# nucypher/SGFHE.jl

Hardware: AMD Instinct MI355X
Metric: bootstraps/sec (higher is better)
Workload: dtype i32

## Files before the change

### sgfhe.jl_amd/csrc/kernels.h

```cpp
#pragma once

#include "ntt.h"

namespace sgfhe {

typedef unsigned __int128 u128;

constexpr int NPR_MAX = 7;
constexpr int LOGE = 4;

struct PrimeK {
    int32_t p;
    uint32_t pinv;
    int32_t sR;
    int32_t sRr;
    uint32_t hoff;
    int32_t r1, r2, r3;
    int32_t qmodp;
    int32_t kappaR;
    int32_t minvR;
    float invp;
    const int32_t *twf;
    const int32_t *twi;
    uint32_t npr;
// ... 131 lines not shown
    static_assert(ROUNDS % 2 == 0, "double rounds");
    const uint32_t s[16] = {0x61707865u, 0x3320646eu, 0x79622d32u, 0x6b206574u,
                            key.k[0], key.k[1], key.k[2], key.k[3],
                            key.k[4], key.k[5], key.k[6], key.k[7], c12, c13, c14, c15};
    uint32_t x[16];
#pragma unroll
    for (int i = 0; i < 16; i++) x[i] = s[i];
#define SGFHE_QR(a, b, c, d)                                                             \
    x[a] += x[b]; x[d] = __builtin_rotateleft32(x[d] ^ x[a], 16);                        \
    x[c] += x[d]; x[b] = __builtin_rotateleft32(x[b] ^ x[c], 12);                        \
    x[a] += x[b]; x[d] = __builtin_rotateleft32(x[d] ^ x[a], 8);                         \
    x[c] += x[d]; x[b] = __builtin_rotateleft32(x[b] ^ x[c], 7);
#pragma unroll
    for (int r = 0; r < ROUNDS / 2; r++) {
        SGFHE_QR(0, 4, 8, 12) SGFHE_QR(1, 5, 9, 13) SGFHE_QR(2, 6, 10, 14) SGFHE_QR(3, 7, 11, 15)
        SGFHE_QR(0, 5, 10, 15) SGFHE_QR(1, 6, 11, 12) SGFHE_QR(2, 7, 8, 13) SGFHE_QR(3, 4, 9, 14)
    }
#undef SGFHE_QR
#pragma unroll
    for (int i = 0; i < 16; i++) out[i] = x[i] + s[i];
}
struct RndRow {
    ChaChaKey key;
    uint32_t call, boot;
};
struct RndArgs {
    ChaChaKey key;
    uint32_t call, chunk;
    const RndRow *rows;
};
template <bool ROWS>
__device__ __forceinline__ void rnd_stream(const RndArgs &ra, uint32_t row, ChaChaKey &key, uint32_t &cz, uint32_t &cw) {
    if constexpr (ROWS) {
        const RndRow r = ra.rows[ra.chunk + row];
        key = r.key; cz = r.boot; cw = r.call;
    } else {
        key = ra.key; cz = ra.chunk + row; cw = ra.call;
    }
}
__device__ __forceinline__ uint4 rnd128(const ChaChaKey &key, uint4 ctr) {
    uint32_t w[16];
    chacha_block<RND_ROUNDS>(key, ctr.x >> 2, ctr.y, ctr.z, ctr.w, w);
    const uint32_t q = ctr.x & 3u;
    return make_uint4(q == 0 ? w[0] : q == 1 ? w[4] : q == 2 ? w[8] : w[12],
                      q == 0 ? w[1] : q == 1 ? w[5] : q == 2 ? w[9] : w[13],
                      q == 0 ? w[2] : q == 1 ? w[6] : q == 2 ? w[10] : w[14],
                      q == 0 ? w[3] : q == 1 ? w[7] : q == 2 ? w[11] : w[15]);
}
__device__ __forceinline__ ulonglong2 random_digits(u128 xn, const CrtConst *CC, const ChaChaKey &key,
                                                    uint4 ctr) {
    const uint4 rv = rnd128(key, ctr);
    const uint64_t span = 2 * CC->xmax + 1;
    const uint64_t r0 = (uint64_t)(((u128)(((uint64_t)rv.y << 32) | rv.x) * span) >> 64);
    const uint64_t r1 = (uint64_t)(((u128)(((uint64_t)rv.w << 32) | rv.z) * span) >> 64);
    const u128 B = CC->B, Q = CC->Q;
    const u128 tsub = mod_wide((u128)r1 * (uint64_t)B + r0, Q, CC->invQ, nullptr);
    const u128 x2 = xn >= tsub ? xn - tsub : xn + Q - tsub;
    uint64_t hi;
    const u128 lo = mod_wide(x2, B, CC->invB, &hi);
    return make_ulonglong2((uint64_t)lo + r0, hi + r1);
}

__device__ __forceinline__ int32_t digit_reduce(uint64_t e, const Mod &md, int32_t sR) {
    return sredc((int64_t)e, md) + sR;
}

__device__ __forceinline__ uint32_t handover_offset(const PrimeK &P) { return 3u * (uint32_t)P.p + P.hoff; }

template <int M, int E>
__device__ __forceinline__ void key_row_products(const int32_t (&x)[1][E], const int32_t *kp, int32_t *zp,
                                                 const Mod &md) {
#pragma unroll
    for (int h = 0; h < E / 4; h++) {
        const int4 a = reinterpret_cast<const int4 *>(kp)[h];
        const int4 bq = reinterpret_cast<const int4 *>(kp + M)[h];
        const int32_t ka[4] = {a.x, a.y, a.z, a.w};
        const int32_t kb[4] = {bq.x, bq.y, bq.z, bq.w};
        int32_t r0[4], r1[4];
#pragma unroll
        for (int t = 0; t < 4; t++) {
            const int32_t u = x[0][4 * h + t];
            r0[t] = smont(u, ka[t], md);
            r1[t] = smont(u, kb[t], md);
        }
        reinterpret_cast<int4 *>(zp)[h] = make_int4(r0[0], r0[1], r0[2], r0[3]);
        reinterpret_cast<int4 *>(zp + M)[h] = make_int4(r1[0], r1[1], r1[2], r1[3]);
    }
}
template <int M>
__device__ __forceinline__ void zpart_sum4(const int32_t *zp, int h, int32_t (&acc)[4]) {
    acc[0] = acc[1] = acc[2] = acc[3] = 0;
#pragma unroll
    for (int ph = 0; ph < 4; ph++) {
        const int4 v = reinterpret_cast<const int4 *>(zp + (size_t)ph * 2 * M)[h];
        acc[0] += v.x; acc[1] += v.y; acc[2] += v.z; acc[3] += v.w;
    }
}

struct QuarterHead {
    uint32_t q;
    int32_t wB, wP;
    __device__ __forceinline__ QuarterHead(uint32_t q_, const PrimeK &P)
        : q(q_), wB((q_ & 2) ? P.f3 : P.f2), wP((q_ & 2) ? P.fp3 : P.fp2) {}
    template <int MS>
    __device__ __forceinline__ int32_t point(const uint32_t *dl, const uint16_t *dh, uint32_t i, const PrimeK &P,
                                             const Mod &md, int32_t sRd) const {
        int32_t X[4];
#pragma unroll
        for (int t = 0; t < 4; t++)
            X[t] = digit_reduce(dl[i + t * MS] | ((uint64_t)dh[i + t * MS] << 32), md, sRd);
        const int32_t u = smont(X[2], P.f1, md);
        const int32_t a = (q & 2) ? X[0] - u : X[0] + u;
        const int32_t w = sredc((int64_t)X[1] * wB + (int64_t)X[3] * wP, md);
        return sred_floor((q & 1) ? a - w : a + w, md);
    }
};

template <int LOGM, int E>
__device__ __forceinline__ void rot_factors(int32_t (&dfac)[E], const PrimeK &P, uint32_t j, uint32_t q, int t) {
    constexpr uint32_t M = 1u << LOGM;
#pragma unroll
    for (int e = 0; e < E; e++) {
        const uint32_t sl = q * (M / 4) + (uint32_t)(E * t + e);
        const uint32_t br = __brev(sl) >> (32 - LOGM);
        dfac[e] = P.pw[(j * (2u * br + 1u)) & (2u * M - 1u)];
    }
}
__device__ __forceinline__ int32_t rot_centre(int32_t dfac, const PrimeK &P, const Mod &md) {
    return scentre(dfac - P.r1, md);
}

template <int NP>
__device__ __forceinline__ void quarter_residues(const int32_t *__restrict__ ypart, PrimeSet PS, uint32_t bc,
                                                 uint32_t i, uint32_t logm, uint32_t (&y)[NP]) {
    const uint32_t MS = (1u << logm) >> 2, jq = i & (MS - 1), qq = i >> (logm - 2);
#pragma unroll
    for (int q = 0; q < NP; q++) {
        const PrimeK P = PS[q];
        const Mod md = mod_of(P);
        const int32_t *yp = ypart + (((size_t)bc * NP + q) * 4) * MS + jq;
        int32_t r;
        if (qq & 1u) {
            const int32_t c1 = smont(yp[0] - yp[MS], P.v2, md), c3 = smont(yp[2 * MS] - yp[3 * MS], P.v3, md);
            r = (qq & 2u) ? smont(c1 - c3, P.v1, md) : c1 + c3;
        } else {
            const int32_t c0 = sred(yp[0] + yp[MS], md), c2 = sred(yp[2 * MS] + yp[3 * MS], md);
            r = (qq & 2u) ? smont(c0 - c2, P.v1, md) : c0 + c2;
        }
        y[q] = (uint32_t)r + handover_offset(P);
    }
}

constexpr int EXT_WAVES = 4;
constexpr int wide_split(int logm) { return logm >= 13 ? 2 : 4; }
constexpr int DET_SPLIT = 0;
constexpr int EXT_LE3_MAX = 9;
template <int LOGM, int LE, bool WIDE = false>
__global__ void __launch_bounds__((NttGeom<LOGM, LE>::T), (NttGeom<LOGM, LE>::T >= 256 ? EXT_WAVES : 1))
k_extprod(const uint64_t *__restrict__ dig, const int32_t *__restrict__ keyk,
          uint32_t *__restrict__ yres, const uint32_t *__restrict__ ua, PrimeSet PS, uint32_t k,
          uint32_t n, uint32_t mode) {
    using G = NttGeom<LOGM, LE>;
    constexpr int M = G::M, T = G::T, E = G::E;
    extern __shared__ __attribute__((aligned(16))) uint32_t lds[];
    int32_t *const z1 = reinterpret_cast<int32_t *>(lds) + M + threadIdx.x;

    const int tid = threadIdx.x;
    const uint32_t g = blockIdx.x;
    const uint32_t slot = g >> 3;
    const uint32_t npr = PS[0].npr;
    const uint32_t b = (slot / npr) * 8 + (g & 7);
    const uint32_t pi = slot % npr;
    const PrimeK P = PS[pi];
    const Mod md = mod_of(P);
    const uint32_t cpad = gridDim.x / npr;
    const BufRsrc rdig = make_rsrc(dig, cpad * 32u * (uint32_t)M);
    const BufRsrc rkey = make_rsrc(keyk, npr * 32u * (uint32_t)M);
#ifdef SGFHE_ABL_NO_YRES
    const BufRsrc ryres = make_rsrc(yres, 0u);
#else
    const BufRsrc ryres = make_rsrc(yres, cpad * npr * 8u * (uint32_t)M);
#endif

    const int32_t sRd = (mode & MODE_RANDOM) ? P.sRr : P.sR;
    constexpr int SPLIT = E == 16 ? (WIDE ? wide_split(LOGM) : DET_SPLIT) : 0;
    int64_t acc0[E];
#pragma unroll
    for (int e = 0; e < E; e++) { acc0[e] = 0; z1[e * T] = 0; }
#pragma unroll 1
    for (int ph = 0; ph < 4; ph++) {
        const int tid = (int)threadIdx.x + (int)opaque_zero();
        int32_t x[1][E];
        const uint32_t srec = (b * 2u + (uint32_t)(ph >> 1)) * 16u * (uint32_t)M;
        const uint32_t slo = srec + (uint32_t)(ph & 1) * 4u * (uint32_t)M;
        const uint32_t shi = srec + 8u * (uint32_t)M + (uint32_t)(ph & 1) * 2u * (uint32_t)M;
        const uint32_t vlo = 4u * (uint32_t)tid, vhi = 2u * (uint32_t)tid;
#pragma unroll
        for (int e = 0; e < E; e++) {
#ifdef SGFHE_ABL_NO_DIG
            x[0][e] = digit_reduce((uint64_t)(tid + e) * 0x9E3779B97F4Aull, md, sRd);
#else
            const uint32_t OL = (uint32_t)(4 * T * e), OH = (uint32_t)(2 * T * e);
            const uint32_t lo = buf_ld_u32(rdig, vlo + (OL & 4095u), slo + (OL & ~4095u));
            uint32_t hi = buf_ld_u16(rdig, vhi + (OH & 4095u), shi + (OH & ~4095u));
            if constexpr (WIDE)
                hi |= buf_ld_u8(rdig, (uint32_t)tid + ((uint32_t)(T * e) & 4095u),
                                srec + 12u * (uint32_t)M + (uint32_t)(ph & 1) * (uint32_t)M + ((uint32_t)(T * e) & ~4095u)) << 16;
            x[0][e] = digit_reduce(lo | ((uint64_t)hi << 32), md, sRd);
#endif
            if constexpr (SPLIT > 1)
                if ((e + 1) % (E / SPLIT) == 0 && e + 1 < E) __builtin_amdgcn_sched_barrier(0);
        }
        SGFHE_SYNC();

        const uint32_t skey = (pi * 8u + (uint32_t)ph * 2u) * 4u * (uint32_t)M;
        const uint32_t vkey = 4u * (uint32_t)E * (uint32_t)tid;
        int4 ka4[E / 4], kb4[E / 4];
        ntt_forward<LOGM, 1, LE>(x, lds, P.twf, tid, md);
#pragma unroll
        for (int h = 0; h < E / 4; h++) {
#ifdef SGFHE_ABL_NO_KEY
            ka4[h] = make_int4(tid, h, ph, 7), kb4[h] = make_int4(h, tid, 5, ph);
#else
            ka4[h] = buf_ld_i4(rkey, vkey + 16u * (uint32_t)h, skey);
            kb4[h] = buf_ld_i4(rkey, vkey + 16u * (uint32_t)h, skey + 4u * (uint32_t)M);
#endif
        }

        const Mod &mdp = md;
#pragma unroll
        for (int h = 0; h < E / 4; h++) {
            const int4 a = ka4[h], bq = kb4[h];
            const int32_t ka[4] = {a.x, a.y, a.z, a.w};
            const int32_t kb[4] = {bq.x, bq.y, bq.z, bq.w};
#pragma unroll
            for (int t = 0; t < 4; t++) {
                const int e = 4 * h + t;
                const int32_t u = x[0][e];
                acc0[e] += (int64_t)u * ka[t];
                int32_t *zp = reinterpret_cast<int32_t *>(lds) + M + e * T + tid;
                *zp += smont(u, kb[t], mdp);
            }
        }
    }
    int32_t z[2][E];
    constexpr bool WIDE0 = !inv_r4(LOGM) && LE == 4 && NttGeom<LOGM, LE>::SLAST_INV >= 0 &&
                           !(NttGeom<LOGM, LE>::RHO == 0 && NttGeom<LOGM, LE>::STOP == 0);
#pragma unroll
    for (int e = 0; e < E; e++) {
        const int32_t r0 = sredc(acc0[e], md);
        z[0][e] = WIDE0 ? r0 : sred(r0, md);
        z[1][e] = sred(z1[e * T], md);
    }
    SGFHE_SYNC();
    ntt_inverse<LOGM, 2, LE, WIDE0>(z, lds, P.twi, tid, md);

    const uint32_t sy0 = (b * 2u * npr + pi) * 4u * (uint32_t)M;
    const uint32_t sy1 = sy0 + npr * 4u * (uint32_t)M;
    const uint32_t vout = 4u * (uint32_t)tid;
    if (mode & MODE_PLAIN) {
#pragma unroll
        for (int c = 0; c < 2; c++)
#pragma unroll
            for (int e = 0; e < E; e++)
                buf_st_u32(ryres, vout + ((uint32_t)(4 * T * e) & 4095u),
                              (c ? sy1 : sy0) + ((uint32_t)(4 * T * e) & ~4095u),
                              condsub(sfull(z[c][e], md) + P.hoff, (uint32_t)P.p));
        return;
    }
    const uint32_t j = ua[(size_t)b * n + k];
    const uint32_t yoff = handover_offset(P);
    lds_store<LOGM, 2, LE, G::STOP>(z, lds, tid);
    SGFHE_SYNC();
    {
        constexpr uint32_t LOWMASK = (1u << G::STOP) - 1u;
        const uint32_t s0 = ((uint32_t)tid - j) & (2 * M - 1);
        const uint32_t lowswz = swz<LE>(s0 & LOWMASK);
        const uint32_t h0 = s0 >> G::STOP;
#pragma unroll
        for (int e = 0; e < E; e++) {
            const uint32_t he = h0 + e;
            const uint32_t hipart = (he & (E - 1)) << G::STOP;
            const uint32_t addr = hipart ^ lowswz ^ (G::STOP >= 9 ? 0u : swz_bits<LE>(hipart));
            const uint32_t smask = 0u - ((he >> LE) & 1u);
            const uint32_t yoe = yoff - smask;
#pragma unroll
            for (int c = 0; c < 2; c++) {
                const uint32_t v = lds[c * M + addr];
                const uint32_t y = (v ^ smask) + (yoe - (uint32_t)z[c][e]);
                buf_st_u32(ryres, vout + ((uint32_t)(4 * T * e) & 4095u),
                              (c ? sy1 : sy0) + ((uint32_t)(4 * T * e) & ~4095u), y);
            }
        }
    }
}

struct U96 {
    uint32_t w0, w1, w2;
};
__device__ __forceinline__ void mad96(U96 &a, uint32_t y, const uint32_t (&c)[3]) {
    const uint64_t p0 = (uint64_t)y * c[0] + a.w0;
    const uint64_t p1 = (uint64_t)y * c[1] + a.w1 + (p0 >> 32);
    a.w0 = (uint32_t)p0;
    a.w1 = (uint32_t)p1;
    a.w2 = y * c[2] + a.w2 + (uint32_t)(p1 >> 32);
}
template <int NP>
__device__ __forceinline__ U96 crt_reduce(const uint32_t (&y)[NP], const CrtConst *__restrict__ CC,
                                          bool have_old, ulonglong2 d) {
    float f = 0.f;
    double Sd = 0.0;
#pragma unroll
    for (int q = 0; q < NP; q++) {
        f += (float)y[q] * CC->invp[q];
#ifndef SGFHE_ABL_CRT_NOSD
        Sd += (double)y[q] * CC->cd[q];
#endif
    }
    const int alpha = (int)f;
    const uint4 tv = *reinterpret_cast<const uint4 *>(CC->T32[alpha]);
    U96 a = {tv.x, tv.y, tv.z};
    Sd += CC->Td[alpha];
#pragma unroll
    for (int q = 0; q < NP; q++) mad96(a, y[q], CC->c32[q]);
    if (have_old) {
        const uint64_t B = (uint64_t)CC->B;
        const uint32_t h0 = (uint32_t)d.y, h1 = (uint32_t)(d.y >> 32);
        const uint32_t b0 = (uint32_t)B, b1 = (uint32_t)(B >> 32);
        const uint64_t p0 = (uint64_t)h0 * b0 + a.w0 + (uint32_t)d.x;
        const uint64_t p1 = (uint64_t)h0 * b1 + (uint64_t)h1 * b0 + a.w1 + (uint32_t)(d.x >> 32) + (p0 >> 32);
        a.w0 = (uint32_t)p0;
        a.w1 = (uint32_t)p1;
        a.w2 += h1 * b1 + (uint32_t)(p1 >> 32);
#ifndef SGFHE_ABL_CRT_NOSD
        Sd += (double)d.y * CC->Bd + (double)d.x;
#endif
    }
    {
        const uint64_t q1 = (uint64_t)(Sd * CC->invQ);
        const uint32_t qa = (uint32_t)q1, qb = (uint32_t)(q1 >> 32);
        const uint64_t m0 = (uint64_t)qa * CC->Q32[0];
        const uint64_t m1 = (uint64_t)qa * CC->Q32[1] + (uint64_t)qb * CC->Q32[0] + (m0 >> 32);
        const uint32_t m2 = qa * CC->Q32[2] + qb * CC->Q32[1] + (uint32_t)(m1 >> 32);
        const uint64_t r0 = (uint64_t)a.w0 - (uint32_t)m0;
        const uint64_t r1 = (uint64_t)a.w1 - (uint32_t)m1 - ((r0 >> 32) & 1u);
        a.w2 = a.w2 - m2 - (uint32_t)((r1 >> 32) & 1u);
        a.w0 = (uint32_t)r0;
        a.w1 = (uint32_t)r1;
    }
    {
        const uint64_t Qlo = ((uint64_t)CC->Q32[1] << 32) | CC->Q32[0];
        const uint32_t Qhi = CC->Q32[2];
        uint64_t lo = ((uint64_t)a.w1 << 32) | a.w0;
        uint32_t hi = a.w2;
        if ((int32_t)hi < 0) {
            const uint64_t nlo = lo + Qlo;
            hi = hi + Qhi + (nlo < lo);
            lo = nlo;
        } else if (hi > Qhi || (hi == Qhi && lo >= Qlo)) {
            const uint64_t nlo = lo - Qlo;
            hi = hi - Qhi - (lo < Qlo);
            lo = nlo;
        }
        a.w0 = (uint32_t)lo;
        a.w1 = (uint32_t)(lo >> 32);
        a.w2 = hi;
    }
    return a;
}
template <int NP, bool ABLATE = false>
__device__ __forceinline__ void load_residues(const uint32_t *__restrict__ yres, uint32_t bc, uint32_t i,
                                              uint32_t logm, uint32_t (&y)[NP]) {
    const uint32_t yo = 4u * ((bc * NP << logm) + i);
#pragma unroll
    for (int q = 0; q < NP; q++) {
#ifdef SGFHE_ABL_NO_YRES
        if constexpr (ABLATE) { y[q] = (((bc << logm) + i) * 2654435761u + (uint32_t)q * 40503u) >> 3; continue; }
#endif
        y[q] = ld_off<uint32_t>(yres, yo + ((uint32_t)(4 * q) << logm));
    }
}
template <int NP, bool ABLATE = false>
__device__ __forceinline__ void load_residues4(const uint32_t *__restrict__ yres, uint32_t bc, uint32_t i,
                                               uint32_t logm, uint4 (&yv)[NP]) {
    typedef unsigned int v4u __attribute__((ext_vector_type(4)));
    const uint32_t yo = 4u * ((bc * NP << logm) + i);
#pragma unroll
    for (int q = 0; q < NP; q++) {
#ifdef SGFHE_ABL_NO_YLOAD
        if constexpr (ABLATE) { yv[q] = make_uint4((((bc << logm) + i) >> 2) + q, yo, i + 7u * q, bc); continue; }
#endif
        const v4u t = __builtin_nontemporal_load(reinterpret_cast<const v4u *>(
            reinterpret_cast<const char *>(yres) + yo + ((uint32_t)(4 * q) << logm)));
        yv[q] = make_uint4(t.x, t.y, t.z, t.w);
    }
}
template <int NP>
__device__ __forceinline__ void residues_of(const uint4 (&yv)[NP], int j, uint32_t (&y)[NP]) {
#pragma unroll
    for (int q = 0; q < NP; q++) y[q] = j == 0 ? yv[q].x : j == 1 ? yv[q].y : j == 2 ? yv[q].z : yv[q].w;
}

template <int NP, bool ROWS = false>
__global__ void __launch_bounds__(256)
k_crt_acc(const uint32_t *__restrict__ yres, uint64_t *__restrict__ dig,
          const CrtConst *__restrict__ CC, uint32_t total, uint32_t logm, uint32_t mode,
          RndArgs ra, uint32_t iter) {
    const uint32_t t = blockIdx.x * 256 + threadIdx.x;
// ... 1304 lines not shown
```

### sgfhe.jl_amd/csrc/ntt.h

```cpp
#pragma once

#include "rns_arith.h"

#ifdef SGFHE_ABL_NO_BARRIER
#define SGFHE_SYNC() ((void)0)
#else
#define SGFHE_SYNC() __syncthreads()
#endif

namespace sgfhe {

constexpr bool fwd_vec4(int logm) { return logm != 12 && logm != 14; }
constexpr bool inv_r4(int logm) { return logm != 12; }

template <int LOGE>
__host__ __device__ constexpr uint32_t swz_bits(uint32_t idx) {
    if constexpr (LOGE == 3)
        return (((idx >> 6) & 1u) * 0x09u) ^ (((idx >> 7) & 1u) * 0x12u) ^ (((idx >> 5) & 1u) * 0x04u);
    else
        return (((idx >> 5) & 1u) * 0x01u) ^ (((idx >> 6) & 1u) * 0x02u) ^
               (((idx >> 7) & 1u) * 0x04u) ^ (((idx >> 8) & 1u) * 0x18u);
}
template <int LOGE>
__host__ __device__ constexpr uint32_t swz(uint32_t idx) { return idx ^ swz_bits<LOGE>(idx); }

template <int LOGM, int LOGE>
struct NttGeom {
    static constexpr int M = 1 << LOGM;
    static constexpr int E = 1 << LOGE;
    static constexpr int T = M / E;
    static constexpr int RHO = LOGM % LOGE;
    static constexpr int STOP = LOGM - LOGE;
    static constexpr int SFIRST = RHO ? LOGM - RHO - LOGE : LOGM - 2 * LOGE;
    static constexpr int SLAST_INV = RHO ? LOGM - RHO - LOGE : STOP;
};

__device__ __forceinline__ uint32_t opaque_zero() {
    uint32_t z = 0;
    asm volatile("" : "+v"(z));
    return z;
}
__device__ __forceinline__ uint32_t opaque_zero_s() {
    uint32_t z = 0;
    asm volatile("" : "+s"(z));
    return z;
}

typedef __attribute__((address_space(4))) int32_t gmem_i32;


template <int LOGM, int LOGE, int S, int BHI, int BLO>
__device__ __forceinline__ void load_twiddles_at(int32_t (&t)[(1 << LOGE) - 1], const gmem_i32 *tw,
                                                 uint32_t hi) {
    constexpr int NG = 1 << (LOGE - 1 - BHI);
    const gmem_i32 *w = tw + (1u << (LOGM - 1 - S - BHI)) + (hi << (LOGE - 1 - BHI));
#pragma unroll
    for (int g = 0; g < NG; g++)
#ifdef SGFHE_ABL_NO_TW
        t[NG - 1 + g] = (int32_t)(hi + g + 12345u);
#else
        t[NG - 1 + g] = w[g];
#endif
    if constexpr (BHI > BLO) load_twiddles_at<LOGM, LOGE, S, BHI - 1, BLO>(t, tw, hi);
}
template <int LOGM, int LOGE, int S, int BHI, int BLO>
__device__ __forceinline__ void load_twiddles(int32_t (&t)[(1 << LOGE) - 1], const int32_t *tw,
                                              uint32_t hi) {
    if constexpr ((1 << S) >= 64) {
        const uint32_t hu = __builtin_amdgcn_readfirstlane(hi);
        load_twiddles_at<LOGM, LOGE, S, BHI, BLO>(t, (const gmem_i32 *)tw + opaque_zero_s(), hu);
    } else {
        load_twiddles_at<LOGM, LOGE, S, BHI, BLO>(t, (const gmem_i32 *)tw, hi);
    }
}


template <int NP, int LOGE, int B>
__device__ __forceinline__ void fwd_stage(int32_t (&x)[NP][1 << LOGE],
                                          const int32_t (&t)[(1 << LOGE) - 1], const Mod &md) {
    constexpr int NG = 1 << (LOGE - 1 - B);
#pragma unroll
    for (int q = 0; q < NP; q++)
#pragma unroll
        for (int g = 0; g < NG; g++)
#pragma unroll
            for (int l = 0; l < (1 << B); l++) {
                const int e0 = (g << (B + 1)) | l;
                bfly_fwd(x[q][e0], x[q][e0 | (1 << B)], t[NG - 1 + g], md);
            }
}
template <int NP, int LOGE, int BH>
__device__ __forceinline__ void fwd_step4(int32_t (&x)[NP][1 << LOGE], const int32_t (&t)[(1 << LOGE) - 1],
                                          const int32_t (&tp)[(1 << LOGE) - 1], const Mod &md) {
    static_assert(BH >= 1, "a radix-4 step covers local bits BH and BH - 1");
    constexpr int NGA = 1 << (LOGE - 1 - BH);
    constexpr int LO = 1 << (BH - 1), HI = 1 << BH;
#pragma unroll
    for (int q = 0; q < NP; q++)
#pragma unroll
        for (int g = 0; g < NGA; g++)
#pragma unroll
            for (int l = 0; l < LO; l++) {
                const int e0 = (g << (BH + 1)) | l;
                const int32_t wA = t[NGA - 1 + g];
                const int32_t wB0 = t[2 * NGA - 1 + 2 * g], wB1 = t[2 * NGA - 1 + 2 * g + 1];
                const int32_t P0 = tp[2 * NGA - 1 + 2 * g], P1 = tp[2 * NGA - 1 + 2 * g + 1];
                const int32_t X0 = x[q][e0], X1 = x[q][e0 | LO], X2 = x[q][e0 | HI], X3 = x[q][e0 | HI | LO];
                const int32_t u = smont(X2, wA, md);
                const int32_t a = X0 + u, b = X0 - u;
                const int32_t s_ = sredc((int64_t)X1 * wB0 + (int64_t)X3 * P0, md);
                const int32_t r_ = sredc((int64_t)X1 * wB1 + (int64_t)X3 * P1, md);
                x[q][e0] = a + s_;
                x[q][e0 | LO] = a - s_;
                x[q][e0 | HI] = b + r_;
                x[q][e0 | HI | LO] = b - r_;
            }
}
template <int NP, int LOGE, int BH>
__device__ __forceinline__ void fwd_reduce_x0(int32_t (&x)[NP][1 << LOGE], const Mod &md) {
#pragma unroll
    for (int q = 0; q < NP; q++)
#pragma unroll
        for (int e = 0; e < (1 << LOGE); e++)
            if ((e & (3 << (BH - 1))) == 0) x[q][e] = sred_floor(x[q][e], md);
}

template <int NP, int LOGE, int B>
__device__ __forceinline__ void inv_step4(int32_t (&x)[NP][1 << LOGE], const int32_t (&t)[(1 << LOGE) - 1],
                                          const int32_t (&tp)[(1 << LOGE) - 1], const Mod &md) {
    constexpr int NGA = 1 << (LOGE - 2 - B);
    constexpr int LO = 1 << B, HI = 1 << (B + 1);
#pragma unroll
    for (int q = 0; q < NP; q++)
#pragma unroll
        for (int g = 0; g < NGA; g++)
#pragma unroll
            for (int l = 0; l < LO; l++) {
                const int e0 = (g << (B + 2)) | l;
                const int32_t wA = t[NGA - 1 + g];
                const int32_t wB0 = t[2 * NGA - 1 + 2 * g], wB1 = t[2 * NGA - 1 + 2 * g + 1];
                const int32_t P0 = tp[2 * NGA - 1 + 2 * g], P1 = tp[2 * NGA - 1 + 2 * g + 1];
                const int32_t x0 = x[q][e0], x1 = x[q][e0 | LO], x2 = x[q][e0 | HI], x3 = x[q][e0 | HI | LO];
                const int32_t s0 = x0 + x1, s1 = x2 + x3, d0 = x0 - x1, d1 = x2 - x3;
                x[q][e0] = s0 + s1;
                x[q][e0 | HI] = smont(s0 - s1, wA, md);
                x[q][e0 | LO] = sredc((int64_t)d0 * wB0 + (int64_t)d1 * wB1, md);
                x[q][e0 | HI | LO] = sredc((int64_t)d0 * P0 + (int64_t)d1 * P1, md);
            }
}
template <int NP, int LOGE, int B>
__device__ __forceinline__ void inv_reduce_y0(int32_t (&x)[NP][1 << LOGE], const Mod &md) {
#pragma unroll
    for (int q = 0; q < NP; q++)
#pragma unroll
        for (int e = 0; e < (1 << LOGE); e++)
            if ((e & (3 << B)) == 0) x[q][e] = sred(x[q][e], md);
}

template <int NP, int LOGE, int B, uint32_t REDMASK, uint32_t REDMASK0>
__device__ __forceinline__ void inv_stage(int32_t (&x)[NP][1 << LOGE],
                                          const int32_t (&t)[(1 << LOGE) - 1], const Mod &md) {
    constexpr int NG = 1 << (LOGE - 1 - B);
#pragma unroll
    for (int q = 0; q < NP; q++)
#pragma unroll
        for (int g = 0; g < NG; g++)
#pragma unroll
            for (int l = 0; l < (1 << B); l++) {
                const int e0 = (g << (B + 1)) | l;
                bfly_inv(x[q][e0], x[q][e0 | (1 << B)], t[NG - 1 + g], md,
                         (((q == 0 ? REDMASK0 : REDMASK) >> e0) & 1u) != 0);
            }
}

template <int NP, int LOGE, int BHI, int BLO>
__device__ __forceinline__ void fwd_stages(int32_t (&x)[NP][1 << LOGE],
                                           const int32_t (&t)[(1 << LOGE) - 1], const Mod &md) {
    fwd_stage<NP, LOGE, BHI>(x, t, md);
    if constexpr (BHI > BLO) fwd_stages<NP, LOGE, BHI - 1, BLO>(x, t, md);
}
template <int NP, int LOGE>
__device__ __forceinline__ void fwd_reduce_x(int32_t (&x)[NP][1 << LOGE], const Mod &md) {
#pragma unroll
    for (int q = 0; q < NP; q++)
#pragma unroll
        for (int e = 0; e < (1 << (LOGE - 1)); e++) x[q][e] = sred_floor(x[q][e], md);
}
template <int LOGE, int B, int BLO, int BHI, int BFIRST, int LASTRED>
constexpr uint32_t inv_red_mask() {
    if (LOGE == 4 && BFIRST == 0 && BHI == 3 && LASTRED) {
        uint32_t m = 0;
        for (int e0 = 0; e0 < 16; e0++) {
            if (e0 & (1 << B)) continue;
            bool red = false;
            if (LASTRED == 3)
                red = B == 0 || B == 3 || (B == 2 && (e0 & 2) == 0);
            else
                red = B == 1 ? (e0 & 1) == 0
                    : B == 2 ? (e0 & 3) == 1
                    : B == 3 ? (LASTRED == 2 ? (e0 == 0 || e0 == 2 || e0 == 3) : true) : false;
            if (red) m |= 1u << e0;
        }
        return m;
    }
    return ((((B - BFIRST) & 1) != 0) || (LASTRED && B == BHI)) ? 0xFFFFFFFFu : 0u;
}
template <int NP, int LOGE, int BLO, int BHI, int BFIRST, int LASTRED, int LASTRED0 = LASTRED>
__device__ __forceinline__ void inv_stages(int32_t (&x)[NP][1 << LOGE],
                                           const int32_t (&t)[(1 << LOGE) - 1], const Mod &md) {
    inv_stage<NP, LOGE, BLO, inv_red_mask<LOGE, BLO, BLO, BHI, BFIRST, LASTRED>(),
              inv_red_mask<LOGE, BLO, BLO, BHI, BFIRST, LASTRED0>()>(x, t, md);
    if constexpr (BLO < BHI) inv_stages<NP, LOGE, BLO + 1, BHI, BFIRST, LASTRED, LASTRED0>(x, t, md);
}


template <int LOGE, int S>
__device__ __forceinline__ uint32_t lds_base(int tid) {
    const uint32_t lo = (uint32_t)tid & ((1u << S) - 1u);
    const uint32_t hi = (uint32_t)tid >> S;
    return swz<LOGE>((hi << (S + LOGE)) | lo);
}
template <int LOGM, int NP, int LOGE, int S>
__device__ __forceinline__ void lds_store(const int32_t (&x)[NP][1 << LOGE], uint32_t *lds, int tid) {
#ifdef SGFHE_ABL_NO_LDS
    return;
#endif
    constexpr int M = 1 << LOGM;
    const uint32_t pb = lds_base<LOGE, S>(tid) << 2;
    char *const base = reinterpret_cast<char *>(lds);
#pragma unroll
    for (int e = 0; e < (1 << LOGE); e++) {
        const uint32_t a = pb ^ (swz<LOGE>((uint32_t)e << S) << 2);
#pragma unroll
        for (int q = 0; q < NP; q++) *reinterpret_cast<int32_t *>(base + q * M * 4 + a) = x[q][e];
    }
}
template <int LOGM, int NP, int LOGE, int S>
__device__ __forceinline__ void lds_load(int32_t (&x)[NP][1 << LOGE], const uint32_t *lds, int tid) {
#ifdef SGFHE_ABL_NO_LDS
    return;
#endif
    constexpr int M = 1 << LOGM;
    const uint32_t pb = lds_base<LOGE, S>(tid) << 2;
    const char *const base = reinterpret_cast<const char *>(lds);
#pragma unroll
    for (int e = 0; e < (1 << LOGE); e++) {
        const uint32_t a = pb ^ (swz<LOGE>((uint32_t)e << S) << 2);
#pragma unroll
        for (int q = 0; q < NP; q++) x[q][e] = *reinterpret_cast<const int32_t *>(base + q * M * 4 + a);
    }
}


template <int LOGE, int SLOW>
__device__ __forceinline__ void exchange_sync() {
#ifdef SGFHE_ABL_ONEBAR
    if constexpr ((SLOW == 0 || SLOW == LOGE) && (1 << LOGE) <= 64) {
#else
    if constexpr (SLOW == 0 && (1 << LOGE) <= 64) {
#endif
#ifndef SGFHE_ABL_NO_BARRIER
        __builtin_amdgcn_fence(__ATOMIC_RELEASE, "wavefront");
#endif
    } else {
        SGFHE_SYNC();
    }
}

template <int LOGM, int NP, int LOGE, int SPREV, int SCUR>
struct FwdPasses {
    static __device__ __forceinline__ void run(int32_t (&x)[NP][1 << LOGE], uint32_t *lds,
                                               const int32_t *tw, int tid, const Mod &md) {
        int32_t t[(1 << LOGE) - 1], tp[(1 << LOGE) - 1];
        load_twiddles<LOGM, LOGE, SCUR, LOGE - 1, 0>(t, tw, (uint32_t)tid >> SCUR);
        constexpr bool UNIFORM = (1 << SCUR) >= 64;
        constexpr bool TWO_STEPS = LOGE == 4 && UNIFORM;
        if constexpr (UNIFORM || fwd_vec4(LOGM)) {
            load_twiddles<LOGM, LOGE, SCUR, LOGE - 2, LOGE - 2>(tp, tw + (2 << LOGM), (uint32_t)tid >> SCUR);
            if constexpr (TWO_STEPS) load_twiddles<LOGM, LOGE, SCUR, 0, 0>(tp, tw + (2 << LOGM), (uint32_t)tid >> SCUR);
        }
        lds_store<LOGM, NP, LOGE, SPREV>(x, lds, tid);
        exchange_sync<LOGE, SCUR>();
        lds_load<LOGM, NP, LOGE, SCUR>(x, lds, tid);
        Mod mdl = md;
        mdl.negp += (int32_t)opaque_zero_s();
        if constexpr (TWO_STEPS) {
            fwd_reduce_x0<NP, LOGE, 3>(x, mdl);
            fwd_step4<NP, LOGE, 3>(x, t, tp, mdl);
            fwd_reduce_x0<NP, LOGE, 1>(x, mdl);
            fwd_step4<NP, LOGE, 1>(x, t, tp, mdl);
        } else if constexpr (UNIFORM || fwd_vec4(LOGM)) {
            fwd_reduce_x<NP, LOGE>(x, mdl);
            fwd_step4<NP, LOGE, LOGE - 1>(x, t, tp, mdl);
            fwd_stages<NP, LOGE, LOGE - 3, 0>(x, t, mdl);
        } else {
            fwd_reduce_x<NP, LOGE>(x, mdl);
            fwd_stages<NP, LOGE, LOGE - 1, 0>(x, t, mdl);
        }
        if constexpr (SCUR >= LOGE)
            FwdPasses<LOGM, NP, LOGE, SCUR, SCUR - LOGE>::run(x, lds, tw, tid, md);
    }
};
template <int LOGM, int LOGE, int S>
__device__ __forceinline__ void load_inv_products(int32_t (&tp)[(1 << LOGE) - 1], const int32_t *tw, int tid) {
    if constexpr (inv_r4(LOGM)) {
        load_twiddles<LOGM, LOGE, S, 0, 0>(tp, tw + (2 << LOGM), (uint32_t)tid >> S);
        if constexpr (LOGE == 4 && (1 << S) >= 64)
            load_twiddles<LOGM, LOGE, S, 2, 2>(tp, tw + (2 << LOGM), (uint32_t)tid >> S);
    }
}
template <int LOGM, int NP, int LOGE, int SCUR, int SLAST, bool FINAL = false, bool WIDE0 = false>
struct InvPasses {
    static __device__ __forceinline__ void run(int32_t (&x)[NP][1 << LOGE], uint32_t *lds,
                                               const int32_t *tw, int tid, const Mod &md,
                                               const int32_t (&t)[(1 << LOGE) - 1],
                                               const int32_t (&tp)[(1 << LOGE) - 1]) {
        constexpr int MODE = (FINAL && SCUR == SLAST) ? 2 : 1;
        if constexpr (!inv_r4(LOGM)) {
            static_assert(!WIDE0 || (LOGE == 4 && !(FINAL && SLAST == 0)), "wide first pass: radix 16, not the final pass");
            inv_stages<NP, LOGE, 0, LOGE - 1, 0, MODE, (WIDE0 && SCUR == 0) ? 3 : MODE>(x, t, md);
        } else {
            static_assert(!WIDE0, "the radix-4 inverse takes every polynomial below 0.75 * 2^29");
            constexpr bool UNIFORM = (1 << SCUR) >= 64;
            inv_step4<NP, LOGE, 0>(x, t, tp, md);
            inv_reduce_y0<NP, LOGE, 0>(x, md);
            if constexpr (LOGE == 4 && UNIFORM) {
                inv_step4<NP, LOGE, 2>(x, t, tp, md);
                inv_reduce_y0<NP, LOGE, 2>(x, md);
            } else if constexpr (LOGE == 4) {
                inv_stage<NP, LOGE, 2, 0u, 0u>(x, t, md);
                inv_stage<NP, LOGE, 3, MODE == 2 ? 0x000Fu : 0x00FFu, MODE == 2 ? 0x000Fu : 0x00FFu>(x, t, md);
            } else {
                static_assert(LOGE == 3, "8 or 16 points per thread");
                inv_stage<NP, LOGE, 2, MODE == 2 ? 0u : 0x0Fu, MODE == 2 ? 0u : 0x0Fu>(x, t, md);
            }
        }
        if constexpr (SCUR < SLAST) {
            int32_t tn[(1 << LOGE) - 1], tpn[(1 << LOGE) - 1];
            load_twiddles<LOGM, LOGE, SCUR + LOGE, LOGE - 1, 0>(tn, tw,
                                                                (uint32_t)tid >> (SCUR + LOGE));
            load_inv_products<LOGM, LOGE, SCUR + LOGE>(tpn, tw, tid);
            lds_store<LOGM, NP, LOGE, SCUR>(x, lds, tid);
            exchange_sync<LOGE, SCUR>();
            lds_load<LOGM, NP, LOGE, SCUR + LOGE>(x, lds, tid);
            InvPasses<LOGM, NP, LOGE, SCUR + LOGE, SLAST, FINAL, WIDE0>::run(x, lds, tw, tid, md, tn, tpn);
        }
    }
};

template <int LOGM, int NP, int LOGE>
__device__ __forceinline__ void ntt_forward(int32_t (&x)[NP][1 << LOGE], uint32_t *lds,
                                            const int32_t *tw, int tid, const Mod &md) {
    using G = NttGeom<LOGM, LOGE>;
    constexpr int BLO = G::RHO == 0 ? 0 : LOGE - G::RHO;
    int32_t t[(1 << LOGE) - 1];
    load_twiddles<LOGM, LOGE, G::STOP, LOGE - 1, BLO>(t, tw, 0u);
    fwd_stages<NP, LOGE, LOGE - 1, BLO>(x, t, md);
    if constexpr (G::SFIRST >= 0)
        FwdPasses<LOGM, NP, LOGE, G::STOP, G::SFIRST>::run(x, lds, tw, tid, md);
}

template <int LOGM, int NP, int LOGE, bool WIDE0 = false>
__device__ __forceinline__ void ntt_inverse(int32_t (&x)[NP][1 << LOGE], uint32_t *lds,
                                            const int32_t *tw, int tid, const Mod &md) {
    using G = NttGeom<LOGM, LOGE>;
    if constexpr (G::RHO == 0) {
        int32_t t[(1 << LOGE) - 1], tp[(1 << LOGE) - 1];
        load_twiddles<LOGM, LOGE, 0, LOGE - 1, 0>(t, tw, (uint32_t)tid);
        load_inv_products<LOGM, LOGE, 0>(tp, tw, tid);
        InvPasses<LOGM, NP, LOGE, 0, G::STOP, true, WIDE0>::run(x, lds, tw, tid, md, t, tp);
    } else {
        int32_t tp[(1 << LOGE) - 1];
        if constexpr (G::SLAST_INV >= 0) {
            int32_t t[(1 << LOGE) - 1], tq[(1 << LOGE) - 1];
            load_twiddles<LOGM, LOGE, 0, LOGE - 1, 0>(t, tw, (uint32_t)tid);
            load_inv_products<LOGM, LOGE, 0>(tq, tw, tid);
            InvPasses<LOGM, NP, LOGE, 0, G::SLAST_INV, false, WIDE0>::run(x, lds, tw, tid, md, t, tq);
            load_twiddles<LOGM, LOGE, G::STOP, LOGE - 1, LOGE - G::RHO>(tp, tw, 0u);
            lds_store<LOGM, NP, LOGE, G::SLAST_INV>(x, lds, tid);
            SGFHE_SYNC();
            lds_load<LOGM, NP, LOGE, G::STOP>(x, lds, tid);
        } else {
            load_twiddles<LOGM, LOGE, G::STOP, LOGE - 1, LOGE - G::RHO>(tp, tw, 0u);
        }
        inv_stages<NP, LOGE, LOGE - G::RHO, LOGE - 1, LOGE - G::RHO, 0>(x, tp, md);
    }
}

}
```

Baseline: 2141.

## Process digit pairs per forward NTT, keep both accumulators in registers

The external-product kernel now loads two digit polynomials per iteration and runs a two-polynomial forward NTT, halving the outer loop from four phases to two. Both output accumulators stay in 32-bit registers, each updated by one Montgomery reduction per pair of products, instead of one 64-bit register accumulator plus one accumulator held in LDS. Key loads are double-buffered in groups with scheduling barriers. The WIDE0 lazy-reduction path in the inverse NTT is removed. This trades LDS traffic and barriers for more register pressure, which may reduce occupancy.

```diff
diff --git a/sgfhe.jl_amd/csrc/kernels.h b/sgfhe.jl_amd/csrc/kernels.h
--- a/sgfhe.jl_amd/csrc/kernels.h
+++ b/sgfhe.jl_amd/csrc/kernels.h
@@ -307,8 +307,7 @@
 }
 
 constexpr int EXT_WAVES = 4;
-constexpr int wide_split(int logm) { return logm >= 13 ? 2 : 4; }
-constexpr int DET_SPLIT = 0;
+constexpr int pair_split(int e, bool wide) { return e == 16 && wide ? 2 : 0; }
 constexpr int EXT_LE3_MAX = 9;
 template <int LOGM, int LE, bool WIDE = false>
 __global__ void __launch_bounds__((NttGeom<LOGM, LE>::T), (NttGeom<LOGM, LE>::T >= 256 ? EXT_WAVES : 1))
@@ -318,7 +317,6 @@
     using G = NttGeom<LOGM, LE>;
     constexpr int M = G::M, T = G::T, E = G::E;
     extern __shared__ __attribute__((aligned(16))) uint32_t lds[];
-    int32_t *const z1 = reinterpret_cast<int32_t *>(lds) + M + threadIdx.x;
 
     const int tid = threadIdx.x;
     const uint32_t g = blockIdx.x;
@@ -338,77 +336,81 @@
 #endif
 
     const int32_t sRd = (mode & MODE_RANDOM) ? P.sRr : P.sR;
-    constexpr int SPLIT = E == 16 ? (WIDE ? wide_split(LOGM) : DET_SPLIT) : 0;
-    int64_t acc0[E];
-#pragma unroll
-    for (int e = 0; e < E; e++) { acc0[e] = 0; z1[e * T] = 0; }
+    constexpr int SPLIT = pair_split(E, WIDE);
+    int32_t acc[2][E];
+#pragma unroll
+    for (int e = 0; e < E; e++) acc[0][e] = acc[1][e] = 0;
 #pragma unroll 1
-    for (int ph = 0; ph < 4; ph++) {
+    for (int pp = 0; pp < 2; pp++) {
         const int tid = (int)threadIdx.x + (int)opaque_zero();
-        int32_t x[1][E];
-        const uint32_t srec = (b * 2u + (uint32_t)(ph >> 1)) * 16u * (uint32_t)M;
-        const uint32_t slo = srec + (uint32_t)(ph & 1) * 4u * (uint32_t)M;
-        const uint32_t shi = srec + 8u * (uint32_t)M + (uint32_t)(ph & 1) * 2u * (uint32_t)M;
+        int32_t x[2][E];
+        const uint32_t srec = (b * 2u + (uint32_t)pp) * 16u * (uint32_t)M;
         const uint32_t vlo = 4u * (uint32_t)tid, vhi = 2u * (uint32_t)tid;
 #pragma unroll
         for (int e = 0; e < E; e++) {
+#pragma unroll
+            for (int r = 0; r < 2; r++) {
 #ifdef SGFHE_ABL_NO_DIG
-            x[0][e] = digit_reduce((uint64_t)(tid + e) * 0x9E3779B97F4Aull, md, sRd);
+                x[r][e] = digit_reduce((uint64_t)(tid + e + 16 * r) * 0x9E3779B97F4Aull, md, sRd);
 #else
-            const uint32_t OL = (uint32_t)(4 * T * e), OH = (uint32_t)(2 * T * e);
-            const uint32_t lo = buf_ld_u32(rdig, vlo + (OL & 4095u), slo + (OL & ~4095u));
-            uint32_t hi = buf_ld_u16(rdig, vhi + (OH & 4095u), shi + (OH & ~4095u));
-            if constexpr (WIDE)
-                hi |= buf_ld_u8(rdig, (uint32_t)tid + ((uint32_t)(T * e) & 4095u),
-                                srec + 12u * (uint32_t)M + (uint32_t)(ph & 1) * (uint32_t)M + ((uint32_t)(T * e) & ~4095u)) << 16;
-            x[0][e] = digit_reduce(lo | ((uint64_t)hi << 32), md, sRd);
+                const uint32_t slo = srec + (uint32_t)r * 4u * (uint32_t)M;
+                const uint32_t shi = srec + 8u * (uint32_t)M + (uint32_t)r * 2u * (uint32_t)M;
+                const uint32_t OL = (uint32_t)(4 * T * e), OH = (uint32_t)(2 * T * e);
+                const uint32_t lo = buf_ld_u32(rdig, vlo + (OL & 4095u), slo + (OL & ~4095u));
+                uint32_t hi = buf_ld_u16(rdig, vhi + (OH & 4095u), shi + (OH & ~4095u));
+                if constexpr (WIDE)
+                    hi |= buf_ld_u8(rdig, (uint32_t)tid + ((uint32_t)(T * e) & 4095u),
+                                    srec + 12u * (uint32_t)M + (uint32_t)r * (uint32_t)M + ((uint32_t)(T * e) & ~4095u)) << 16;
+                x[r][e] = digit_reduce(lo | ((uint64_t)hi << 32), md, sRd);
 #endif
+            }
             if constexpr (SPLIT > 1)
                 if ((e + 1) % (E / SPLIT) == 0 && e + 1 < E) __builtin_amdgcn_sched_barrier(0);
         }
         SGFHE_SYNC();
 
-        const uint32_t skey = (pi * 8u + (uint32_t)ph * 2u) * 4u * (uint32_t)M;
+        ntt_forward<LOGM, 2, LE>(x, lds, P.twf, tid, md);
+        const uint32_t skey = (pi * 8u + (uint32_t)pp * 4u) * 4u * (uint32_t)M;
         const uint32_t vkey = 4u * (uint32_t)E * (uint32_t)tid;
-        int4 ka4[E / 4], kb4[E / 4];
-        ntt_forward<LOGM, 1, LE>(x, lds, P.twf, tid, md);
+
+        __builtin_amdgcn_sched_barrier(0);
+        int4 kq[2][2][2];
+        const auto key_group = [&](int4 (&kg)[2][2], int h) {
+#pragma unroll
+            for (int r = 0; r < 2; r++)
+#pragma unroll
+                for (int c = 0; c < 2; c++)
+#ifdef SGFHE_ABL_NO_KEY
+                    kg[r][c] = make_int4(tid + r, h + c, pp, 7);
+#else
+                    kg[r][c] = buf_ld_i4(rkey, vkey + 16u * (uint32_t)h, skey + (uint32_t)(2 * r + c) * 4u * (uint32_t)M);
+#endif
+        };
+        key_group(kq[0], 0);
 #pragma unroll
         for (int h = 0; h < E / 4; h++) {
-#ifdef SGFHE_ABL_NO_KEY
-            ka4[h] = make_int4(tid, h, ph, 7), kb4[h] = make_int4(h, tid, 5, ph);
-#else
-            ka4[h] = buf_ld_i4(rkey, vkey + 16u * (uint32_t)h, skey);
-            kb4[h] = buf_ld_i4(rkey, vkey + 16u * (uint32_t)h, skey + 4u * (uint32_t)M);
-#endif
+            if (h + 1 < E / 4) key_group(kq[(h + 1) & 1], h + 1);
+            const int4 (&kg)[2][2] = kq[h & 1];
+#pragma unroll
+            for (int c = 0; c < 2; c++) {
+                const int32_t k0[4] = {kg[0][c].x, kg[0][c].y, kg[0][c].z, kg[0][c].w};
+                const int32_t k1[4] = {kg[1][c].x, kg[1][c].y, kg[1][c].z, kg[1][c].w};
+#pragma unroll
+                for (int t = 0; t < 4; t++) {
+                    const int e = 4 * h + t;
+                    acc[c][e] += sredc((int64_t)x[0][e] * k0[t] + (int64_t)x[1][e] * k1[t], md);
+                }
+            }
+            __builtin_amdgcn_sched_barrier(0);
         }
-
-        const Mod &mdp = md;
-#pragma unroll
-        for (int h = 0; h < E / 4; h++) {
-            const int4 a = ka4[h], bq = kb4[h];
-            const int32_t ka[4] = {a.x, a.y, a.z, a.w};
-            const int32_t kb[4] = {bq.x, bq.y, bq.z, bq.w};
-#pragma unroll
-            for (int t = 0; t < 4; t++) {
-                const int e = 4 * h + t;
-                const int32_t u = x[0][e];
-                acc0[e] += (int64_t)u * ka[t];
-                int32_t *zp = reinterpret_cast<int32_t *>(lds) + M + e * T + tid;
-                *zp += smont(u, kb[t], mdp);
-            }
-        }
     }
     int32_t z[2][E];
-    constexpr bool WIDE0 = !inv_r4(LOGM) && LE == 4 && NttGeom<LOGM, LE>::SLAST_INV >= 0 &&
-                           !(NttGeom<LOGM, LE>::RHO == 0 && NttGeom<LOGM, LE>::STOP == 0);
 #pragma unroll
     for (int e = 0; e < E; e++) {
-        const int32_t r0 = sredc(acc0[e], md);
-        z[0][e] = WIDE0 ? r0 : sred(r0, md);
-        z[1][e] = sred(z1[e * T], md);
-    }
-    SGFHE_SYNC();
-    ntt_inverse<LOGM, 2, LE, WIDE0>(z, lds, P.twi, tid, md);
+        z[0][e] = sred(acc[0][e], md);
+        z[1][e] = sred(acc[1][e], md);
+    }
+    ntt_inverse<LOGM, 2, LE>(z, lds, P.twi, tid, md);
 
     const uint32_t sy0 = (b * 2u * npr + pi) * 4u * (uint32_t)M;
     const uint32_t sy1 = sy0 + npr * 4u * (uint32_t)M;
diff --git a/sgfhe.jl_amd/csrc/ntt.h b/sgfhe.jl_amd/csrc/ntt.h
--- a/sgfhe.jl_amd/csrc/ntt.h
+++ b/sgfhe.jl_amd/csrc/ntt.h
@@ -157,7 +157,7 @@
             if ((e & (3 << B)) == 0) x[q][e] = sred(x[q][e], md);
 }
 
-template <int NP, int LOGE, int B, uint32_t REDMASK, uint32_t REDMASK0>
+template <int NP, int LOGE, int B, uint32_t REDMASK>
 __device__ __forceinline__ void inv_stage(int32_t (&x)[NP][1 << LOGE],
                                           const int32_t (&t)[(1 << LOGE) - 1], const Mod &md) {
     constexpr int NG = 1 << (LOGE - 1 - B);
@@ -169,7 +169,7 @@
             for (int l = 0; l < (1 << B); l++) {
                 const int e0 = (g << (B + 1)) | l;
                 bfly_inv(x[q][e0], x[q][e0 | (1 << B)], t[NG - 1 + g], md,
-                         (((q == 0 ? REDMASK0 : REDMASK) >> e0) & 1u) != 0);
+                         ((REDMASK >> e0) & 1u) != 0);
             }
 }
 
@@ -192,25 +192,20 @@
         uint32_t m = 0;
         for (int e0 = 0; e0 < 16; e0++) {
             if (e0 & (1 << B)) continue;
-            bool red = false;
-            if (LASTRED == 3)
-                red = B == 0 || B == 3 || (B == 2 && (e0 & 2) == 0);
-            else
-                red = B == 1 ? (e0 & 1) == 0
-                    : B == 2 ? (e0 & 3) == 1
-                    : B == 3 ? (LASTRED == 2 ? (e0 == 0 || e0 == 2 || e0 == 3) : true) : false;
+            const bool red = B == 1 ? (e0 & 1) == 0
+                           : B == 2 ? (e0 & 3) == 1
+                           : B == 3 ? (LASTRED == 2 ? (e0 == 0 || e0 == 2 || e0 == 3) : true) : false;
             if (red) m |= 1u << e0;
         }
         return m;
     }
     return ((((B - BFIRST) & 1) != 0) || (LASTRED && B == BHI)) ? 0xFFFFFFFFu : 0u;
 }
-template <int NP, int LOGE, int BLO, int BHI, int BFIRST, int LASTRED, int LASTRED0 = LASTRED>
+template <int NP, int LOGE, int BLO, int BHI, int BFIRST, int LASTRED>
 __device__ __forceinline__ void inv_stages(int32_t (&x)[NP][1 << LOGE],
                                            const int32_t (&t)[(1 << LOGE) - 1], const Mod &md) {
-    inv_stage<NP, LOGE, BLO, inv_red_mask<LOGE, BLO, BLO, BHI, BFIRST, LASTRED>(),
-              inv_red_mask<LOGE, BLO, BLO, BHI, BFIRST, LASTRED0>()>(x, t, md);
-    if constexpr (BLO < BHI) inv_stages<NP, LOGE, BLO + 1, BHI, BFIRST, LASTRED, LASTRED0>(x, t, md);
+    inv_stage<NP, LOGE, BLO, inv_red_mask<LOGE, BLO, BLO, BHI, BFIRST, LASTRED>()>(x, t, md);
+    if constexpr (BLO < BHI) inv_stages<NP, LOGE, BLO + 1, BHI, BFIRST, LASTRED>(x, t, md);
 }
 
 
@@ -309,7 +304,7 @@
             load_twiddles<LOGM, LOGE, S, 2, 2>(tp, tw + (2 << LOGM), (uint32_t)tid >> S);
     }
 }
-template <int LOGM, int NP, int LOGE, int SCUR, int SLAST, bool FINAL = false, bool WIDE0 = false>
+template <int LOGM, int NP, int LOGE, int SCUR, int SLAST, bool FINAL = false>
 struct InvPasses {
     static __device__ __forceinline__ void run(int32_t (&x)[NP][1 << LOGE], uint32_t *lds,
                                                const int32_t *tw, int tid, const Mod &md,
@@ -317,10 +312,8 @@
                                                const int32_t (&tp)[(1 << LOGE) - 1]) {
         constexpr int MODE = (FINAL && SCUR == SLAST) ? 2 : 1;
         if constexpr (!inv_r4(LOGM)) {
-            static_assert(!WIDE0 || (LOGE == 4 && !(FINAL && SLAST == 0)), "wide first pass: radix 16, not the final pass");
-            inv_stages<NP, LOGE, 0, LOGE - 1, 0, MODE, (WIDE0 && SCUR == 0) ? 3 : MODE>(x, t, md);
+            inv_stages<NP, LOGE, 0, LOGE - 1, 0, MODE>(x, t, md);
         } else {
-            static_assert(!WIDE0, "the radix-4 inverse takes every polynomial below 0.75 * 2^29");
             constexpr bool UNIFORM = (1 << SCUR) >= 64;
             inv_step4<NP, LOGE, 0>(x, t, tp, md);
             inv_reduce_y0<NP, LOGE, 0>(x, md);
@@ -328,11 +321,11 @@
                 inv_step4<NP, LOGE, 2>(x, t, tp, md);
                 inv_reduce_y0<NP, LOGE, 2>(x, md);
             } else if constexpr (LOGE == 4) {
-                inv_stage<NP, LOGE, 2, 0u, 0u>(x, t, md);
-                inv_stage<NP, LOGE, 3, MODE == 2 ? 0x000Fu : 0x00FFu, MODE == 2 ? 0x000Fu : 0x00FFu>(x, t, md);
+                inv_stage<NP, LOGE, 2, 0u>(x, t, md);
+                inv_stage<NP, LOGE, 3, MODE == 2 ? 0x000Fu : 0x00FFu>(x, t, md);
             } else {
                 static_assert(LOGE == 3, "8 or 16 points per thread");
-                inv_stage<NP, LOGE, 2, MODE == 2 ? 0u : 0x0Fu, MODE == 2 ? 0u : 0x0Fu>(x, t, md);
+                inv_stage<NP, LOGE, 2, MODE == 2 ? 0u : 0x0Fu>(x, t, md);
             }
         }
         if constexpr (SCUR < SLAST) {
@@ -343,7 +336,7 @@
             lds_store<LOGM, NP, LOGE, SCUR>(x, lds, tid);
             exchange_sync<LOGE, SCUR>();
             lds_load<LOGM, NP, LOGE, SCUR + LOGE>(x, lds, tid);
-            InvPasses<LOGM, NP, LOGE, SCUR + LOGE, SLAST, FINAL, WIDE0>::run(x, lds, tw, tid, md, tn, tpn);
+            InvPasses<LOGM, NP, LOGE, SCUR + LOGE, SLAST, FINAL>::run(x, lds, tw, tid, md, tn, tpn);
         }
     }
 };
@@ -360,7 +353,7 @@
         FwdPasses<LOGM, NP, LOGE, G::STOP, G::SFIRST>::run(x, lds, tw, tid, md);
 }
 
-template <int LOGM, int NP, int LOGE, bool WIDE0 = false>
+template <int LOGM, int NP, int LOGE>
 __device__ __forceinline__ void ntt_inverse(int32_t (&x)[NP][1 << LOGE], uint32_t *lds,
                                             const int32_t *tw, int tid, const Mod &md) {
     using G = NttGeom<LOGM, LOGE>;
@@ -368,14 +361,14 @@
         int32_t t[(1 << LOGE) - 1], tp[(1 << LOGE) - 1];
         load_twiddles<LOGM, LOGE, 0, LOGE - 1, 0>(t, tw, (uint32_t)tid);
         load_inv_products<LOGM, LOGE, 0>(tp, tw, tid);
-        InvPasses<LOGM, NP, LOGE, 0, G::STOP, true, WIDE0>::run(x, lds, tw, tid, md, t, tp);
+        InvPasses<LOGM, NP, LOGE, 0, G::STOP, true>::run(x, lds, tw, tid, md, t, tp);
     } else {
         int32_t tp[(1 << LOGE) - 1];
         if constexpr (G::SLAST_INV >= 0) {
             int32_t t[(1 << LOGE) - 1], tq[(1 << LOGE) - 1];
             load_twiddles<LOGM, LOGE, 0, LOGE - 1, 0>(t, tw, (uint32_t)tid);
             load_inv_products<LOGM, LOGE, 0>(tq, tw, tid);
-            InvPasses<LOGM, NP, LOGE, 0, G::SLAST_INV, false, WIDE0>::run(x, lds, tw, tid, md, t, tq);
+            InvPasses<LOGM, NP, LOGE, 0, G::SLAST_INV, false>::run(x, lds, tw, tid, md, t, tq);
             load_twiddles<LOGM, LOGE, G::STOP, LOGE - 1, LOGE - G::RHO>(tp, tw, 0u);
             lds_store<LOGM, NP, LOGE, G::SLAST_INV>(x, lds, tid);
             SGFHE_SYNC();
```

After: 2138. Within noise of the previous version (-0.2%).
